# MiniMax-AI/VTP

Hardware: AMD Instinct MI355X
Metric: images/sec/node VTP-B f16d64 256x256 train step (higher is better)
Workload: dtype bf16

## Files before the change

### include/vtp_hip.h

```cpp
#ifndef VTP_HIP_H
#define VTP_HIP_H
#ifdef __cplusplus
extern "C" {
#endif

#define VTP_ABI_VERSION 1

int vtp_abi_version(void);
const char* vtp_last_error(void);

enum { VTP_EPI_BF16 = 0, VTP_EPI_F32 = 1, VTP_EPI_SWIGLU = 2, VTP_EPI_GELU = 3, VTP_EPI_F32_ATOMIC = 4, VTP_EPI_F32_SLAB = 5,
       VTP_EPI_QUICK_GELU = 8 };
int vtp_gemm_splits(int K, int splits);
int vtp_gemm_tn_splits(int M, int N, int K);
int vtp_gemm_tn(const void* A, int lda, const void* B, int ldb, void* C, int ldc, int ldc2, const float* resid, int M, int N,
                int K, int epilogue, int a_grp, int a_pre, int b_grp, int b_pre, int c_grp, int c_pre, int splits,
                float* a_colsum, void* stream);
int vtp_gemm_tn_grouped(const void* probs, int nprob, int ntiles, int K, int splits, void* part, void* ticket, void* stream);
int vtp_gemm_tn_grouped_limit(const void* probs, int nprob, int ntiles, int K, const int* k_rows, void* stream);
int vtp_gemm_tn_grouped_items(const void* probs, int nprob, int ntiles, int K, const void* items, int nitems, int slots, void* part,
                              void* ticket, void* stream);
int vtp_set_gemm_tuning(int force_cfg, int xcd_swizzle);
int vtp_set_gemm_dynamic(int on);
int vtp_gemm_debug(void* timing, int grid_limit, int delay_ticks);
// ... 139 lines not shown
int vtp_clip_grad_rows(const float* G, const float* B, const float* logit_scale, float* out, int M, int N, int D, int accumulate,
                       void* stream);
int vtp_clip_grad_cols(const float* G, const float* A, const float* logit_scale, float* out, int M, int N, int D, int accumulate,
                       void* stream);
int vtp_siglip_pairs(float* logits, const float* logit_bias, int B_local, int B_all, int label_offset, float weight,
                     float* loss_sum, float* d_logit_scale, float* d_logit_bias, void* stream);
int vtp_koleo(const float* xn, int* nn_scratch, float* d_xn, float* loss_sum, int B, int D, float weight, float eps, void* stream);
int vtp_sinkhorn_knopp(const void* logits, float inv_temp, void* probs, float* u, float* v, float* scratch, int T, int K, float count,
                       const float* count_dev, const int* n_rows_dev, int n_iters, int phase, void* stream);

int vtp_norm_fwd_e4m3(const float* x, const float* w, const float* b, void* y8, const float* q_scale, float* stats, int M, int D,
                      float eps, int kind, void* stream);
int vtp_quantize_e4m3(const void* src, int src_is_f32, void* dst, long n, const float* scale_dev, float scale, void* stream);
int vtp_amax(const void* src, int src_is_f32, long n, float* amax, void* stream);
int vtp_dequantize_e4m3(const void* src, float* dst, long n, float inv_scale, void* stream);
int vtp_gemm_nt_fp8(const void* A8, int lda, const void* B8, int ldb, void* C, int ldc, void* C2, int ldc2, const float* bias,
                    const float* resid, int M, int N, int K, int epilogue, float alpha, const int* rope_pos, const void* rope_sin,
                    const void* rope_cos, int rope_cols, void* stream);

int vtp_u8_to_images(const void* u8_nhwc, float* img_nchw, long B, int H, int W, const float* mean3, const float* std3, int flip,
                     void* stream);
int vtp_images_to_u8(const float* img_nchw, void* u8_nhwc, long B, int H, int W, const float* sub3, const float* div3, void* stream);
int vtp_latent_channel_stats(const float* latents, double* sums, long B, int C, int hw, void* stream);

int vtp_gather_token_rows(const void* src, const int* idx, void* dst, int T, int D, void* stream);
int vtp_scatter_token_rows(const void* d_dst, const int* idx, void* d_src, int T, int D, void* stream);
int vtp_weight_norm_prep(const float* v, const float* g, void* weff, void* weffT, float* inv_norm, int K, int C, void* stream);
int vtp_weight_norm_bwd(const float* dW, const float* v, const float* g, const float* inv_norm, float* dv, float* dg, int K, int C,
                        void* stream);
int vtp_softmax_center(const void* logits, const float* center, float inv_temp, void* probs, int T, int K, void* stream);
int vtp_softmax_center_dev(const void* logits, const float* center, const float* inv_temp, void* probs, int T, int K, void* stream);
int vtp_dino_ce(const void* student_logits, const void* teacher_probs, const int* t_idx0, const int* t_idx1,
                const float* row_weight, float inv_temp, float* loss_sum, void* d_student_logits, int T, int K, void* stream);
int vtp_center_ema(float* center, const float* col_sum, float inv_count, const float* count_ptr, float momentum, int K,
                   void* stream);

int vtp_conv3x3(const void* x, const void* w, const float* bias, void* y, const void* relu_mask, int NB, int H, int W, int Cin,
                int Cout, int taps, int mode, void* stream);
int vtp_lpips_unfold3(const void* tok, const float* img, void* out, int n, int H, int W, const float* shift, const float* scale,
                      void* stream);
int vtp_lpips_fold3_bwd(const void* dA, void* dt, int n, int H, int W, const float* scale, void* stream);
int vtp_maxpool2_fwd(const void* in, void* out, int NB, int H, int W, int C, void* stream);
int vtp_maxpool2_bwd(const void* Y, const void* dP, const void* tap, void* dY, int NB, int H, int W, int C, void* stream);
int vtp_lpips_tap(const void* f0, const void* f1, const float* w, float* val, void* df0, int n, int H, int W, int C,
                  float gscale, void* stream);

int vtp_probe_logits(const float* X, int ldx, const float* W, const float* bias, float* logits, int ldl, int B, int N, int K,
                     void* stream);
int vtp_probe_ce(const float* logits, int ldl, const long* labels, int B, int H, int C, float inv_rows, float* loss, int* correct,
                 float* dlogits, void* stream);
int vtp_probe_sgd(float* W, float* bias, float* mW, float* mb, const float* dlogits, int ldl, const float* X, int ldx, const float* lr,
                  int B, int H, int C, int K, float momentum, void* stream);

int vtp_zs_class_mean(const float* feat, int ldf, float* Wt, int ldw, int C, int T, int D, float eps, void* stream);
int vtp_zs_topk(const float* F, int ldf, const float* Wt, int ldw, const long* targets, float scale, int B, int C, int D,
                long* counts, int* per_class, int* rank, int* pred, float* logits, int ldl, void* stream);

int vtp_recon_scratch_doubles(long B, int H, int W);
int vtp_recon_metrics(const float* images, const float* recon, long B, int H, int W, const float* sub3, const float* div3,
                      void* ref_u8, void* rec_u8, float* ref_lp, float* rec_lp, double* scratch, long scratch_len, void* stream);
int vtp_recon_finalize(const double* scratch, long scratch_len, long B, int H, int W, float* psnr, float* ssim, double* sse,
                       const float* lpips, double* acc, void* stream);

int vtp_augment_scratch_floats(long N, int S);
int vtp_augment_crops(const void* src_u8, long B, int Hs, int Ws, const float* table, long N, int S, const float* mean3,
                      const float* std3, float* out, float* scratch, long scratch_len, void* stream);
// ... 68 lines not shown
```

### vtp_amd/_lib.py

```python
import ctypes
import os
from ctypes import c_char_p, c_float, c_int, c_long, c_void_p

_HERE = os.path.dirname(os.path.abspath(__file__))
LIB_PATH = os.environ.get("VTP_HIP_LIB") or os.path.join(_HERE, "lib", "libvtp_hip.so")

_P, _I, _L, _F = c_void_p, c_int, c_long, c_float

SIGNATURES = {
    "vtp_gemm_nt": [_P, _I, _P, _I, _P, _I, _P, _I, _P, _P, _P, _I, _I, _I, _I, _I, _I, _I, _I, _I, _F, _P],
    "vtp_norm_fwd": [_P, _P, _P, _P, _P, _I, _I, _F, _I, _P],
    "vtp_norm_bwd": [_P, _P, _P, _P, _P, _P, _P, _P, _P, _P, _I, _I, _I, _P],
    "vtp_norm_bwd_pvec": [_P, _P, _P, _P, _P, _P, _P, _P, _P, _P, _P, _I, _I, _I, _I, _I, _I, _P],
    "vtp_norm_bwd_rows": [_P, _P, _P, _P, _P, _P, _I, _P, _P, _P, _P, _P, _I, _I, _I, _P],
    "vtp_pool_patch_rows": [_P, _P, _I, _I, _I, _F, _P],
    "vtp_rope_qk": [_P, _P, _P, _I, _I, _I, _I, _I, _P],
    "vtp_attn_fwd": [_P, _P, _P, _P, _P, _I, _I, _I, _L, _L, _L, _L, _F, _I, _P],
    "vtp_attn_bwd": [_P, _P, _P, _P, _P, _P, _P, _P, _P, _P, _P, _P, _I, _I, _I, _I, _L, _L, _L, _L, _F, _I, _P],
    "vtp_im2col16": [_P, _P, _I, _I, _I, _P],
    "vtp_im2col16_rows": [_P, _P, _I, _I, _I, _I, _P],
    "vtp_col2im16": [_P, _P, _I, _I, _I, _P],
    "vtp_assemble_tokens": [_P, _P, _P, _P, _I, _I, _I, _P],
    "vtp_transpose_bf16": [_P, _I, _P, _I, _P, _I, _I, _I, _I, _I, _P],
    "vtp_strided_rowsum": [_P, _L, _P, _I, _I, _P],
# ... 23 lines not shown
    "vtp_colsum_bf16": [_P, _I, _P, _I, _I, _I, _I, _I, _P],
    "vtp_colsum_bf16_rows": [_P, _I, _P, _P, _I, _I, _P],
    "vtp_gather_image_rows": [_P, _P, _P, _P, _I, _L, _I, _F, _P],
    "vtp_scatter_image_rows": [_P, _P, _P, _I, _L, _I, _F, _I, _P],
    "vtp_gather_tail_rows": [_P, _P, _P, _P, _P, _I, _I, _I, _I, _P],
    "vtp_tail_row_map": [_P, _P, _I, _I, _I, _P],
    "vtp_expand_rows_bf16": [_P, _P, _P, _I, _I, _I, _P],
    "vtp_layerscale_wgrad": [_P, _P, _P, _P, _P, _P, _P, _P, _I, _I, _P],
    "vtp_scaled_transpose": [_P, _P, _P, _I, _I, _P],
    "vtp_qk_norm_fwd": [_P, _P, _P, _P, _P, _L, _I, _F, _P],
    "vtp_qk_norm_bwd": [_P, _P, _P, _P, _P, _P, _P, _L, _I, _P],
    "vtp_set_gemm_tuning": [_I, _I],
    "vtp_gemm_nt_config": [_I, _I, _I, _I],
    "vtp_gemm_debug": [_P, _I, _I],
    "vtp_attn_debug": [_P, _I, _I, _I],
    "vtp_cu_thief": [_I, _I, _P, _P],
    "vtp_set_gemm_dynamic": [_I],
    "vtp_norm_fwd_e4m3": [_P, _P, _P, _P, _P, _P, _I, _I, _F, _I, _P],
    "vtp_quantize_e4m3": [_P, _I, _P, _L, _P, _F, _P],
    "vtp_amax": [_P, _I, _L, _P, _P],
    "vtp_dequantize_e4m3": [_P, _P, _L, _F, _P],
    "vtp_gemm_nt_fp8": [_P, _I, _P, _I, _P, _I, _P, _I, _P, _P, _I, _I, _I, _I, _F, _P, _P, _P, _I, _P],
    "vtp_u8_to_images": [_P, _P, _L, _I, _I, _P, _P, _I, _P],
    "vtp_images_to_u8": [_P, _P, _L, _I, _I, _P, _P, _P],
    "vtp_latent_channel_stats": [_P, _P, _L, _I, _I, _P],
    "vtp_ema": [_P, _P, _L, _F, _P],
    "vtp_gather_token_rows": [_P, _P, _P, _I, _I, _P],
    "vtp_scatter_token_rows": [_P, _P, _P, _I, _I, _P],
    "vtp_weight_norm_prep": [_P, _P, _P, _P, _P, _I, _I, _P],
    "vtp_weight_norm_bwd": [_P, _P, _P, _P, _P, _P, _I, _I, _P],
    "vtp_softmax_center": [_P, _P, _F, _P, _I, _I, _P],
    "vtp_softmax_center_dev": [_P, _P, _P, _P, _I, _I, _P],
    "vtp_dino_ce": [_P, _P, _P, _P, _P, _F, _P, _P, _I, _I, _P],
    "vtp_center_ema": [_P, _P, _F, _P, _F, _I, _P],
    "vtp_conv3x3": [_P, _P, _P, _P, _P, _I, _I, _I, _I, _I, _I, _I, _P],
    "vtp_lpips_unfold3": [_P, _P, _P, _I, _I, _I, _P, _P, _P],
    "vtp_lpips_fold3_bwd": [_P, _P, _I, _I, _I, _P, _P],
    "vtp_maxpool2_fwd": [_P, _P, _I, _I, _I, _I, _P],
    "vtp_maxpool2_bwd": [_P, _P, _P, _P, _I, _I, _I, _I, _P],
    "vtp_lpips_tap": [_P, _P, _P, _P, _P, _I, _I, _I, _I, _F, _P],
    "vtp_ema_dev": [_P, _P, _L, _P, _P],
    "vtp_adamw_ema_dev": [_P, _P, _P, _P, _P, _P, _L, _P, _P],
    "vtp_adamw_dev_grouped": [_P, _P, _P, _P, _P, _P, _P, _I, _L, _P, _P],
    "vtp_adamw_ema_dev_grouped": [_P, _P, _P, _P, _P, _P, _P, _I, _L, _P, _P],
    "vtp_sumsq_partials_count": [_L],
    "vtp_sumsq_partials": [_P, _L, _P, _P],
    "vtp_sum_partials": [_P, _I, _P, _P],
    "vtp_grad_clip_finalize": [_P, _I, _P, _P, _P, _P],
    "vtp_grad_clip_finalize_guarded": [_P, _I, _P, _P, _P, _P, _P, _P],
    "vtp_adamw_dev_guarded": [_P, _P, _P, _P, _P, _P, _P, _I, _L, _P, _P, _P],
    "vtp_adamw_ema_dev_guarded": [_P, _P, _P, _P, _P, _P, _P, _I, _L, _P, _P, _P],
    "vtp_ema_dev_guarded": [_P, _P, _L, _P, _P, _P],
    "vtp_embed_tokens": [_P, _P, _P, _P, _P, _I, _I, _I, _P],
    "vtp_embed_tokens_bwd": [_P, _P, _P, _P, _I, _I, _I, _P],
    "vtp_gather_rows": [_P, _P, _P, _I, _I, _I, _P],
    "vtp_scatter_rows": [_P, _P, _P, _P, _I, _I, _I, _P],
    "vtp_text_row_plan": [_P, _P, _P, _P, _I, _I, _P],
    "vtp_embed_tokens_packed": [_P, _P, _P, _P, _P, _I, _I, _I, _P],
    "vtp_embed_tokens_bwd_packed": [_P, _P, _P, _P, _P, _I, _I, _I, _P],
    "vtp_gather_rows_packed": [_P, _P, _P, _I, _I, _P],
    "vtp_scatter_rows_packed": [_P, _P, _P, _P, _I, _I, _I, _P],
    "vtp_gelu_bwd_limit": [_P, _P, _P, _I, _I, _I, _P, _P],
    "vtp_norm_fwd_limit": [_P, _P, _P, _P, _P, _I, _I, _F, _I, _P, _P],
    "vtp_norm_bwd_limit": [_P, _P, _P, _P, _P, _P, _P, _P, _P, _P, _I, _I, _I, _P, _P],
    "vtp_gemm_nt_limit": [_P, _I, _P, _I, _P, _I, _P, _I, _P, _P, _P, _I, _I, _I, _I, _F, _P, _P],
    "vtp_attn_fwd_varlen": [_P, _P, _P, _P, _P, _P, _I, _I, _I, _L, _L, _F, _P],
# ... 92 lines not shown
```

### vtp_amd/csrc/ssl.hip

```cpp
#include "common.h"
#include "vtp_hip.h"

namespace vtp {

__global__ __launch_bounds__(256) void gather_token_rows_kernel(const bf16* __restrict__ src, const int* __restrict__ idx,
                                                                bf16* __restrict__ dst, int T, int D) {
  const int d8 = D / 8;
  const long total = (long)T * d8;
  for (long i = blockIdx.x * 256L + threadIdx.x; i < total; i += (long)gridDim.x * 256L) {
    const int t = (int)(i / d8), c = (int)(i % d8);
    const int r = idx[t];
    bf16x8 v;
    if (r >= 0) {
      v = *(const bf16x8*)(src + (long)r * D + 8 * c);
    } else {
#pragma unroll
      for (int e = 0; e < 8; ++e) v[e] = (bf16)0.f;
    }
    *(bf16x8*)(dst + (long)t * D + 8 * c) = v;
  }
}

__global__ __launch_bounds__(256) void scatter_token_rows_kernel(const bf16* __restrict__ d_dst, const int* __restrict__ idx,
                                                                 bf16* __restrict__ d_src, int T, int D) {
// ... 26 lines not shown
    if (weffT) weffT[(long)c * K + k] = w;
  }
  if (lane == 0) inv_norm[k] = inv;
}

__global__ __launch_bounds__(256) void weight_norm_prep_tiled_kernel(const float* __restrict__ v, const float* __restrict__ g,
                                                                     bf16* __restrict__ weff, bf16* __restrict__ weffT,
                                                                     float* __restrict__ inv_norm, int K, int C) {
  __shared__ bf16 tile[64][256 + 2];
  const int lane = threadIdx.x & 63, wave = threadIdx.x >> 6;
  const int k0 = blockIdx.x * 64;
  for (int r = wave; r < 64; r += 4) {
    const int k = k0 + r;
    if (k >= K) break;
    float s = 0.f;
    for (int c = lane; c < C; c += 64) {
      const float x = v[(long)k * C + c];
      s += x * x;
    }
    s = wave_sum(s);
    const float inv = rsqrtf(s);
    const float sc = g[k] * inv;
    for (int c = lane; c < C; c += 64) {
      const bf16 w = f2bf(v[(long)k * C + c] * sc);
      weff[(long)k * C + c] = w;
      tile[r][c] = w;
    }
    if (lane == 0) inv_norm[k] = inv;
  }
  __syncthreads();
  const int k = k0 + lane;
  if (k < K)
    for (int c = wave; c < C; c += 4) weffT[(long)c * K + k] = tile[lane][c];
}

__global__ __launch_bounds__(256) void weight_norm_bwd_kernel(const float* __restrict__ dW, const float* __restrict__ v,
                                                              const float* __restrict__ g, const float* __restrict__ inv_norm,
                                                              float* __restrict__ dv, float* __restrict__ dg, int K, int C) {
  const int lane = threadIdx.x & 63;
  const int k = blockIdx.x * 4 + (threadIdx.x >> 6);
  if (k >= K) return;
  const float inv = inv_norm[k];
  float dot = 0.f;
  for (int c = lane; c < C; c += 64) dot += dW[(long)k * C + c] * v[(long)k * C + c] * inv;
  dot = wave_sum(dot);
  const float sc = g[k] * inv;
  for (int c = lane; c < C; c += 64) {
    const float vh = v[(long)k * C + c] * inv;
    dv[(long)k * C + c] += sc * (dW[(long)k * C + c] - dot * vh);
  }
  if (lane == 0) dg[k] += dot;
}

__device__ __forceinline__ void row_lse(const bf16* __restrict__ row, const float* __restrict__ center, float sc, int K,
                                        float* red, float& mx_out, float& se_out) {
  float mx = -INFINITY, se = 0.f;
  for (int k = threadIdx.x * 8; k < K; k += 256 * 8) {
    bf16x8 v = *(const bf16x8*)(row + k);
#pragma unroll
    for (int e = 0; e < 8; ++e) {
      const float x = (bf2f(v[e]) - (center ? center[k + e] : 0.f)) * sc;
      if (x > mx) {
        se = se * __expf(mx - x) + 1.f;
        mx = x;
      } else {
        se += __expf(x - mx);
      }
    }
  }
#pragma unroll
  for (int o = 32; o > 0; o >>= 1) {
    const float m2 = __shfl_xor(mx, o, 64), s2 = __shfl_xor(se, o, 64);
    const float m = fmaxf(mx, m2);
    se = (mx == -INFINITY ? 0.f : se * __expf(mx - m)) + (m2 == -INFINITY ? 0.f : s2 * __expf(m2 - m));
    mx = m;
  }
  const int w = threadIdx.x >> 6;
  __syncthreads();
  if ((threadIdx.x & 63) == 0) {
    red[2 * w] = mx;
    red[2 * w + 1] = se;
  }
  __syncthreads();
  float m = fmaxf(fmaxf(red[0], red[2]), fmaxf(red[4], red[6]));
  float s = 0.f;
#pragma unroll
// ... 97 lines not shown
  if (wr == 0.f || i0 < 0) {
    for (int k = threadIdx.x * 8; k < K; k += 256 * 8) {
      bf16x8 z;
#pragma unroll
      for (int e = 0; e < 8; ++e) z[e] = (bf16)0.f;
      *(bf16x8*)(drow + k) = z;
    }
    return;
  }
  float mx, se;
  row_lse(row, nullptr, inv_temp, K, red, mx, se);
  const float lse = mx + __logf(se);
  const float nt = i1 >= 0 ? 2.f : 1.f;
  const bf16* p0 = P + (long)i0 * K;
  const bf16* p1 = i1 >= 0 ? P + (long)i1 * K : nullptr;
  float loss = 0.f;
  for (int k = threadIdx.x * 8; k < K; k += 256 * 8) {
    bf16x8 s = *(const bf16x8*)(row + k), a = *(const bf16x8*)(p0 + k), b, o;
    if (p1) b = *(const bf16x8*)(p1 + k);
#pragma unroll
    for (int e = 0; e < 8; ++e) {
      const float lsm = bf2f(s[e]) * inv_temp - lse;
      const float q = bf2f(a[e]) + (p1 ? bf2f(b[e]) : 0.f);
      loss -= q * lsm;
      o[e] = f2bf(wr * inv_temp * (nt * __expf(lsm) - q));
    }
    *(bf16x8*)(drow + k) = o;
  }
  __shared__ float red2[4];
  loss = block_sum<4>(loss, red2);
  if (threadIdx.x == 0) unsafeAtomicAdd(loss_sum, wr * loss);
}

__global__ __launch_bounds__(256) void center_ema_kernel(float* __restrict__ center, const float* __restrict__ col_sum,
                                                         float inv_count, const float* __restrict__ count_ptr, float momentum,
                                                         int K) {
  const int k = blockIdx.x * 256 + threadIdx.x;
  if (count_ptr) inv_count = 1.f / fmaxf(count_ptr[0], 1.f);
  if (k < K) center[k] = momentum * center[k] + (1.f - momentum) * col_sum[k] * inv_count;
}

}
using namespace vtp;

static inline int ssl_grid(long items) {
  long b = (items + 255) / 256;
  return (int)(b > 4096 ? 4096 : (b < 1 ? 1 : b));
}

extern "C" int vtp_gather_token_rows(const void* src, const int* idx, void* dst, int T, int D, void* stream) {
  VTP_REQUIRE(src && idx && dst && T > 0 && D > 0 && D % 8 == 0, "vtp_gather_token_rows: bad argument (D %% 8 == 0)");
  hipLaunchKernelGGL(gather_token_rows_kernel, dim3(ssl_grid((long)T * D / 8)), dim3(256), 0, (hipStream_t)stream,
                     (const bf16*)src, idx, (bf16*)dst, T, D);
  return check_launch("gather_token_rows");
}

extern "C" int vtp_scatter_token_rows(const void* d_dst, const int* idx, void* d_src, int T, int D, void* stream) {
  VTP_REQUIRE(d_dst && idx && d_src && T > 0 && D > 0 && D % 8 == 0, "vtp_scatter_token_rows: bad argument (D %% 8 == 0)");
  hipLaunchKernelGGL(scatter_token_rows_kernel, dim3(ssl_grid((long)T * D / 8)), dim3(256), 0, (hipStream_t)stream,
                     (const bf16*)d_dst, idx, (bf16*)d_src, T, D);
  return check_launch("scatter_token_rows");
}

extern "C" int vtp_weight_norm_prep(const float* v, const float* g, void* weff, void* weffT, float* inv_norm, int K, int C,
                                    void* stream) {
  VTP_REQUIRE(v && g && weff && inv_norm && K > 0 && C > 0, "vtp_weight_norm_prep: bad argument");
  if (weffT && C <= 256)
    hipLaunchKernelGGL(weight_norm_prep_tiled_kernel, dim3(cdiv(K, 64)), dim3(256), 0, (hipStream_t)stream, v, g, (bf16*)weff,
                       (bf16*)weffT, inv_norm, K, C);
  else
    hipLaunchKernelGGL(weight_norm_prep_kernel, dim3(cdiv(K, 4)), dim3(256), 0, (hipStream_t)stream, v, g, (bf16*)weff,
                       (bf16*)weffT, inv_norm, K, C);
  return check_launch("weight_norm_prep");
}

extern "C" int vtp_weight_norm_bwd(const float* dW, const float* v, const float* g, const float* inv_norm, float* dv, float* dg,
                                   int K, int C, void* stream) {
  VTP_REQUIRE(dW && v && g && inv_norm && dv && dg && K > 0 && C > 0, "vtp_weight_norm_bwd: bad argument");
  hipLaunchKernelGGL(weight_norm_bwd_kernel, dim3(cdiv(K, 4)), dim3(256), 0, (hipStream_t)stream, dW, v, g, inv_norm, dv, dg, K, C);
  return check_launch("weight_norm_bwd");
}

static int launch_softmax_center(const void* logits, const float* center, float inv_temp, const float* inv_temp_dev, void* probs, int T,
                                 int K, void* stream) {
  if (K <= 65536 && K >= 8192)
    hipLaunchKernelGGL(softmax_center_reg_kernel, dim3(T), dim3(1024), 0, (hipStream_t)stream, (const bf16*)logits, center,
                       inv_temp, (bf16*)probs, K, inv_temp_dev);
  else
    hipLaunchKernelGGL(softmax_center_kernel, dim3(T), dim3(256), 0, (hipStream_t)stream, (const bf16*)logits, center, inv_temp,
                       (bf16*)probs, K, inv_temp_dev);
  return check_launch("softmax_center");
}

extern "C" int vtp_softmax_center(const void* logits, const float* center, float inv_temp, void* probs, int T, int K,
                                  void* stream) {
  VTP_REQUIRE(logits && probs && T > 0 && K > 0 && K % 8 == 0, "vtp_softmax_center: bad argument (K %% 8 == 0)");
  return launch_softmax_center(logits, center, inv_temp, nullptr, probs, T, K, stream);
}

extern "C" int vtp_softmax_center_dev(const void* logits, const float* center, const float* inv_temp, void* probs, int T, int K,
                                      void* stream) {
  VTP_REQUIRE(logits && probs && inv_temp && T > 0 && K > 0 && K % 8 == 0, "vtp_softmax_center_dev: bad argument (K %% 8 == 0)");
  return launch_softmax_center(logits, center, 0.f, inv_temp, probs, T, K, stream);
}

extern "C" int vtp_dino_ce(const void* student_logits, const void* teacher_probs, const int* t_idx0, const int* t_idx1,
                           const float* row_weight, float inv_temp, float* loss_sum, void* d_student_logits, int T, int K,
                           void* stream) {
  VTP_REQUIRE(student_logits && teacher_probs && t_idx0 && t_idx1 && row_weight && loss_sum && d_student_logits,
              "vtp_dino_ce: null pointer");
  VTP_REQUIRE(T > 0 && K > 0 && K % 8 == 0, "vtp_dino_ce: bad shape (K %% 8 == 0)");
  hipLaunchKernelGGL(dino_ce_kernel, dim3(T), dim3(256), 0, (hipStream_t)stream, (const bf16*)student_logits,
                     (const bf16*)teacher_probs, t_idx0, t_idx1, row_weight, inv_temp, loss_sum, (bf16*)d_student_logits, K);
  return check_launch("dino_ce");
}

extern "C" int vtp_center_ema(float* center, const float* col_sum, float inv_count, const float* count_ptr, float momentum,
                              int K, void* stream) {
  VTP_REQUIRE(center && col_sum && K > 0, "vtp_center_ema: bad argument");
  hipLaunchKernelGGL(center_ema_kernel, dim3(cdiv(K, 256)), dim3(256), 0, (hipStream_t)stream, center, col_sum, inv_count,
                     count_ptr, momentum, K);
  return check_launch("center_ema");
}
```

### vtp_amd/ops.py

```python
from __future__ import annotations

import torch

from . import _lib

EPI_BF16, EPI_F32, EPI_SWIGLU, EPI_GELU, EPI_F32_ATOMIC, EPI_F32_SLAB = 0, 1, 2, 3, 4, 5
EPI_QUICK_GELU = 8
NORM_RMS, NORM_LN = 0, 1


def _s():
    return torch.cuda.current_stream().cuda_stream


def _p(t):
    return 0 if t is None else t.data_ptr()


def _lib_():
    return _lib.load()


def pad8(n: int) -> int:
    return (n + 7) // 8 * 8
# ... 497 lines not shown
def sinkhorn_knopp(logits, inv_temp, probs, u, v, scratch, T, K, count, n_iters=3, phase=-1, count_dev=None, n_rows_dev=None):
    _lib.check(_lib_().vtp_sinkhorn_knopp(_p(logits), inv_temp, _p(probs), _p(u), _p(v), _p(scratch), T, K, float(count), _p(count_dev),
                                          _p(n_rows_dev), n_iters, phase, _s()), "vtp_sinkhorn_knopp")


def gather_token_rows(src, idx, dst, T, D):
    _lib.check(_lib_().vtp_gather_token_rows(_p(src), _p(idx), _p(dst), T, D, _s()), "vtp_gather_token_rows")


def scatter_token_rows(d_dst, idx, d_src, T, D):
    _lib.check(_lib_().vtp_scatter_token_rows(_p(d_dst), _p(idx), _p(d_src), T, D, _s()), "vtp_scatter_token_rows")


def weight_norm_prep(v, g, weff, weffT, inv_norm, K, C):
    _lib.check(_lib_().vtp_weight_norm_prep(_p(v), _p(g), _p(weff), _p(weffT), _p(inv_norm), K, C, _s()), "vtp_weight_norm_prep")


def weight_norm_bwd(dW, v, g, inv_norm, dv, dg, K, C):
    _lib.check(_lib_().vtp_weight_norm_bwd(_p(dW), _p(v), _p(g), _p(inv_norm), _p(dv), _p(dg), K, C, _s()), "vtp_weight_norm_bwd")


def softmax_center(logits, center, inv_temp, probs, T, K):
    if isinstance(inv_temp, torch.Tensor):
        _lib.check(_lib_().vtp_softmax_center_dev(_p(logits), _p(center), _p(inv_temp), _p(probs), T, K, _s()), "vtp_softmax_center_dev")
    else:
        _lib.check(_lib_().vtp_softmax_center(_p(logits), _p(center), inv_temp, _p(probs), T, K, _s()), "vtp_softmax_center")


def dino_ce(s_logits, t_probs, t0, t1, w, inv_temp, loss_sum, d_logits, T, K):
    _lib.check(_lib_().vtp_dino_ce(_p(s_logits), _p(t_probs), _p(t0), _p(t1), _p(w), inv_temp, _p(loss_sum), _p(d_logits), T, K,
                                   _s()), "vtp_dino_ce")


def center_ema(center, col_sum, inv_count, momentum, K, count=None):
    _lib.check(_lib_().vtp_center_ema(_p(center), _p(col_sum), inv_count, _p(count), momentum, K, _s()), "vtp_center_ema")


def ema_dev(t, s, n, momentum_dev):
    _lib.check(_lib_().vtp_ema_dev(_p(t), _p(s), n, _p(momentum_dev), _s()), "vtp_ema_dev")


def adamw_ema_dev(p, g, m, v, teacher, n, hyper, nodecay4=None):
    _lib.check(_lib_().vtp_adamw_ema_dev(_p(p), _p(g), _p(m), _p(v), _p(teacher), _p(nodecay4), n, _p(hyper), _s()), "vtp_adamw_ema_dev")



def adamw_dev_grouped(p, g, m, v, p_bf16, n, hyper, group4, group_tab, ngroups):
    _lib.check(_lib_().vtp_adamw_dev_grouped(_p(p), _p(g), _p(m), _p(v), _p(p_bf16), _p(group4), _p(group_tab), ngroups, n, _p(hyper),
                                             _s()), "vtp_adamw_dev_grouped")


def adamw_ema_dev_grouped(p, g, m, v, teacher, n, hyper, group4, group_tab, ngroups):
    _lib.check(_lib_().vtp_adamw_ema_dev_grouped(_p(p), _p(g), _p(m), _p(v), _p(teacher), _p(group4), _p(group_tab), ngroups, n,
                                                 _p(hyper), _s()), "vtp_adamw_ema_dev_grouped")


def sumsq_partials_count(n: int) -> int:
    return int(_lib_().vtp_sumsq_partials_count(n))


def sumsq_partials(g, n, partials):
    _lib.check(_lib_().vtp_sumsq_partials(_p(g), n, _p(partials), _s()), "vtp_sumsq_partials")


def sum_partials(partials, count, out):
    _lib.check(_lib_().vtp_sum_partials(_p(partials), count, _p(out), _s()), "vtp_sum_partials")
# ... 615 lines not shown
```

### vtp_amd/train.py

```python
from __future__ import annotations

import math
import os
from typing import List, Optional, Sequence, Tuple

import torch

from . import ops
from .engine import BF, F32, OVERLAP


class GradBucketer:

    def __init__(self, flat_g: torch.Tensor, group=None, shard: bool = False, grad_dtype: torch.dtype = torch.float32,
                 force: bool = False):
        import torch.distributed as dist
        self.dist = dist
        self.flat_g = flat_g
        self.group = group
        self.world = dist.get_world_size(group) if dist.is_available() and dist.is_initialized() else 1
        self.rank = dist.get_rank(group) if self.world > 1 else 0
        self.active = self.world > 1 or (bool(force) and dist.is_available() and dist.is_initialized())
        self.works = []
        self.reduced_elems = 0
# ... 355 lines not shown
        if no_decay is not None:
            flags = torch.zeros(st.numel // 4, dtype=torch.uint8)
            for name, (o, k) in st.offsets.items():
                if no_decay(name, tuple(st.params[name].shape)):
                    flags[o // 4:(o + (k + 3) // 4 * 4) // 4] = 1
            self.nodecay4 = flags.to(st.device)
        self.param_groups = self.group_tab = self._group4 = self._group_ring = None
        if param_groups is not None:
            shapes = {name: tuple(st.params[name].shape) for name in st.offsets}
            self.param_groups, rows = resolve_param_groups(param_groups, shapes, no_decay)
            idx = torch.zeros(st.numel // 4, dtype=torch.uint8)
            for name, (o, k) in st.offsets.items():
                idx[o // 4:(o + (k + 3) // 4 * 4) // 4] = rows[name]
            self._group4 = idx.to(st.device)
            self.group_tab = torch.tensor(group_table(self.param_groups), dtype=F32, device=st.device).view(-1, 2)
        self.step_no = 0
        self.loss_sum = torch.zeros(1, dtype=F32, device=st.device)
        self.clip_loss_sum = torch.zeros(1, dtype=F32, device=st.device)
        if shard_optimizer is None:
            shard_optimizer = os.environ.get("VTP_SHARD_OPT", "0") == "1"
        if grad_dtype not in ("fp32", "bf16"):
            raise ValueError(f"grad_dtype must be 'fp32' or 'bf16', got {grad_dtype!r}")
        if grad_dtype == "bf16" and not shard_optimizer:
            raise ValueError("grad_dtype='bf16' needs shard_optimizer=True (the all-reduce path reduces the flat fp32 buffer in place)")
        self.bucketer = GradBucketer(st.flat_g, group, shard=shard_optimizer, grad_dtype=BF if grad_dtype == "bf16" else F32,
                                     force=force_collectives)
        self.shard_optimizer = self.bucketer.shard
        self._shard_layout = None
        self.overlap_opt = (not self.shard_optimizer) and os.environ.get("VTP_OPT_OVERLAP", "1") not in ("0", "false", "off")
        self._opt_stream = self._zero_stream = None
        self._opt_plans = {}
        self._opt_busy = self._zero_busy = False
        self.head_overlap = os.environ.get("VTP_HEAD_OVERLAP", "1") not in ("0", "false", "off")
        self._head_stream, self._head_keys = None, []
        self._works_prev = []
        self.collectives = self.bucketer.active
        if self.collectives:
            from . import _lib
            _lib.load().vtp_set_gemm_dynamic(1)
        self.time_comm = False
        self._comm_events = []
        self.world, self.rank, self.group = self.bucketer.world, self.bucketer.rank, group
        for eng in self._aug_engines():
            eng.rope_aug.reseed(drop_seed, self.rank)
        self._graph_aug = {}
        self.bucket_blocks = bucket_blocks
        self._bucket_plan = self._plan_buckets()
        self.hyper = torch.zeros(16, dtype=F32, device=st.device)
        self.momentum_dev = self.hyper[9:10]
        self._clip = max_grad_norm is not None
        self._max_grad_norm = _max_norm_value(max_grad_norm) if self._clip else None
        self.grad_norm = self.grad_clip_coef = self._clip_partials = self._clip_sum = None
        self._clip_ranges, self._clip_cursor, self._clip_keys = {}, 0, []
        if self._clip:
            self.grad_norm = torch.zeros(1, dtype=F32, device=st.device)
            self.grad_clip_coef = torch.zeros(1, dtype=F32, device=st.device)
            cap = ops.sumsq_partials_count(st.numel) + len(st.offsets)
            self._clip_partials = torch.zeros(cap, dtype=torch.float64, device=st.device)
            self._clip_sum = torch.zeros(1, dtype=torch.float64, device=st.device)
        self._skip_state = self.step_skipped = self.skipped_steps = None
        if self._skip:
            self._skip_state = torch.zeros(4, dtype=torch.int32, device=st.device)
            self.skipped_steps = self._skip_state[1:2]
            self.step_skipped = self._skip_state[2:3]
        self._hyper_ring = None
        self.use_graphs = use_graphs
# ... 81 lines not shown
        return result

    def _ssl_gen(self, P, lead_images=None):
        from .vtp import ssl_forward
        out = ssl_forward(self.model, P["global"], P["local"], P["masks"], P["plan"], P["dev"], train=True, lead_images=lead_images,
                          tail_rows="student_tail_src" in P["dev"])
        self._zero_join()
        if not (self.head_overlap and not self.collectives and OVERLAP.enabled):
            yield from self._ssl_tail(out, P)
            return out
        main = torch.cuda.current_stream()
        self.trunk.d_xnf_buffer(out["ctx"]).zero_()
        if self._head_stream is None:
            self._head_stream = torch.cuda.Stream()
        self._head_stream.wait_stream(main)
        with torch.cuda.stream(self._head_stream), OVERLAP.lane(2):
            was, OVERLAP.enabled = OVERLAP.enabled, False
            try:
                for ev in self._ssl_tail(out, P, zero_dxnf=False):
                    if callable(ev):
                        raise RuntimeError("head stream: the SSL tail asked for a collective")
                    self._head_keys += ev
            finally:
                OVERLAP.enabled = was
        return out

    def _ssl_tail(self, out, P, zero_dxnf: bool = True):
        model, st, head = self.model, self.store, self.ssl_head
        dist = self.bucketer.dist
        K, D = head.K, self.trunk.D
        Tt, Ts, Tm, B2, nl = out["Tt"], out["Ts"], out["Tm"], out["B2"], out["nl"]
        ws = out["ws"]
        t_logits, s_logits = out["teacher_logits"], out["student_logits"]
        probs = ws.get("probs", (Tt, K), BF)
        if self.centering == "sinkhorn_knopp":
            yield from self._sinkhorn_targets(ws, t_logits, probs, P, B2, Tm, K)
        else:
            inv_tt = self.hyper[8:9]
            ops.softmax_center(t_logits, self.center_dino, inv_tt, probs, B2, K)
            ops.softmax_center(t_logits[B2:], self.center_ibot, inv_tt, probs[B2:], Tm, K)
            stats = self.center_stats
            stats.zero_()
            ops.colsum_bf16(t_logits, K, stats, B2, K)
            ops.colsum_bf16_rows(t_logits[B2:], K, stats[K:], P["dev"]["n_masked_i"], Tm, K)
            stats[2 * K:2 * K + 1].copy_(P["dev"]["n_masked_f"])

            def apply_centers():
                ops.center_ema(self.center_dino, stats, 1.0 / (B2 * self.world), self.center_momentum, K)
                ops.center_ema(self.center_ibot, stats[K:], 0.0, self.center_momentum, K, count=stats[2 * K:])
            if self.collectives:
                yield lambda: self.bucketer.works.append((dist.all_reduce(stats, group=self.group, async_op=True), None))
                self._deferred.append(apply_centers)
            else:
                apply_centers()
        d_logits = ws.get("d_logits", (Ts, K), BF)
        ops.dino_ce(s_logits, probs, P["dev"]["t0"], P["dev"]["t1"], P["dev"]["w"], 1.0 / self.student_temp, self.ssl_loss_sum,
                    d_logits, Ts, K)
        dX = head.backward(d_logits, out["head_ctx"])
        if self.koleo_weight > 0:
            self._koleo(ws, out["Hs"], dX, nl, B2, head.Din)
        yield ["dino_head"]
        from .vtp import ssl_head_input_bwd
        dX = ssl_head_input_bwd(model, out, dX)
        ctx = out["ctx"]
        d_xnf = self.trunk.d_xnf_buffer(ctx)
        if zero_dxnf:
            d_xnf.zero_()
        if out["tail"] is not None:
            ops.gather_token_rows(dX, P["dev"]["student_tail_keep"], d_xnf[out["tail"]:], Ts, D)
            return
        seg_g, seg_l = ctx.segs[-2], ctx.segs[-1]
        ops.scatter_token_rows(dX, P["dev"]["student_local_src"], d_xnf[seg_l.row0:], nl, D)
        ops.scatter_token_rows(dX[nl:], P["dev"]["student_global_src"], d_xnf[seg_g.row0:], Ts - nl, D)

    def _sinkhorn_targets(self, ws, t_logits, probs, P, B2, Tm, K):
        dist = self.bucketer.dist
        it = self.sk_iterations
        inv_t = 1.0 / self.teacher_temp
        for tag, lg, pr, T, cnt_dev, rows_dev, count in (("cls", t_logits, probs, B2, None, None, float(B2 * self.world)),
                                                         ("patch", t_logits[B2:], probs[B2:], Tm, P["dev"]["n_masked_f"],
                                                          P["dev"]["n_masked_i"], 0.0)):
            u, v = ws.get(f"sk.u.{tag}", (T,), F32), ws.get(f"sk.v.{tag}", (K,), F32)
            scr = ws.get(f"sk.s.{tag}", (8 + K + T,), F32)
            if not self.collectives:
                ops.sinkhorn_knopp(lg, inv_t, pr, u, v, scr, T, K, count, it, -1, cnt_dev, rows_dev)
                continue
            if cnt_dev is not None:
                gcnt = ws.get("sk.cnt", (1,), F32)
                gcnt.copy_(cnt_dev)
                yield lambda gcnt=gcnt: dist.all_reduce(gcnt, group=self.group)
# ... 767 lines not shown
```

Measured before the change: 760.7.

## Fuse iBOT teacher softmax into CE kernel and add row-wise weight-norm kernels

Adds a fused iBOT cross-entropy kernel that computes the centered teacher softmax inline per masked-token row, instead of first writing a probs buffer for the masked tokens and reading it back in the CE pass. DINO CLS rows still go through the existing softmax_center and dino_ce. It also adds new weight-norm prep and backward kernels that process several rows per wave, stage the transpose through LDS, and use vector stores. The weight-norm kernels are on by default for C<=256 and can be turned off by environment variable. This cuts HBM traffic and kernel launches in the SSL head, at the cost of high register pressure from a 1024-thread kernel that holds 64 logits per thread.

New measurement: 767.2 (median of 6 runs). No clear change (+0.9%).

```diff
diff --git a/include/vtp_hip.h b/include/vtp_hip.h
--- a/include/vtp_hip.h
+++ b/include/vtp_hip.h
@@ -195,6 +195,9 @@
 int vtp_softmax_center_dev(const void* logits, const float* center, const float* inv_temp, void* probs, int T, int K, void* stream);
 int vtp_dino_ce(const void* student_logits, const void* teacher_probs, const int* t_idx0, const int* t_idx1,
                 const float* row_weight, float inv_temp, float* loss_sum, void* d_student_logits, int T, int K, void* stream);
+int vtp_ibot_ce_fused(const void* student_logits, const void* teacher_logits, const float* center, const float* teacher_inv_temp,
+                      const int* t_idx0, const float* row_weight, float inv_temp, float* loss_sum, void* d_student_logits, int T,
+                      int K, void* stream);
 int vtp_center_ema(float* center, const float* col_sum, float inv_count, const float* count_ptr, float momentum, int K,
                    void* stream);
 
diff --git a/vtp_amd/_lib.py b/vtp_amd/_lib.py
--- a/vtp_amd/_lib.py
+++ b/vtp_amd/_lib.py
@@ -79,6 +79,7 @@
     "vtp_softmax_center": [_P, _P, _F, _P, _I, _I, _P],
     "vtp_softmax_center_dev": [_P, _P, _P, _P, _I, _I, _P],
     "vtp_dino_ce": [_P, _P, _P, _P, _P, _F, _P, _P, _I, _I, _P],
+    "vtp_ibot_ce_fused": [_P, _P, _P, _P, _P, _P, _F, _P, _P, _I, _I, _P],
     "vtp_center_ema": [_P, _P, _F, _P, _F, _I, _P],
     "vtp_conv3x3": [_P, _P, _P, _P, _P, _I, _I, _I, _I, _I, _I, _I, _P],
     "vtp_lpips_unfold3": [_P, _P, _P, _I, _I, _I, _P, _P, _P],
diff --git a/vtp_amd/csrc/ssl.hip b/vtp_amd/csrc/ssl.hip
--- a/vtp_amd/csrc/ssl.hip
+++ b/vtp_amd/csrc/ssl.hip
@@ -82,6 +82,73 @@
   const int k = k0 + lane;
   if (k < K)
     for (int c = wave; c < C; c += 4) weffT[(long)c * K + k] = tile[lane][c];
+}
+
+constexpr int WN_ROWS = 128, WN_LD = WN_ROWS + 4;
+__global__ __launch_bounds__(256) void weight_norm_prep_rows_kernel(const float* __restrict__ v, const float* __restrict__ g,
+                                                                    bf16* __restrict__ weff, bf16* __restrict__ weffT,
+                                                                    float* __restrict__ inv_norm, int K, int C) {
+  __shared__ __attribute__((aligned(16))) bf16 tile[256 * WN_LD];
+  const int lane = threadIdx.x & 63, wave = threadIdx.x >> 6;
+  const int k0 = blockIdx.x * WN_ROWS;
+  const int kw = k0 + wave * (WN_ROWS / 4);
+  float x[2][4][4];
+  auto load4 = [&](int b, int kb) {
+#pragma unroll
+    for (int i = 0; i < 4; ++i)
+#pragma unroll
+      for (int j = 0; j < 4; ++j) {
+        const int c = lane + 64 * j;
+        x[b][i][j] = (kb + i < K && c < C) ? v[(long)(kb + i) * C + c] : 0.f;
+      }
+  };
+  load4(0, kw);
+#pragma unroll
+  for (int it = 0; it < WN_ROWS / 16; ++it) {
+    const int kb = kw + 4 * it, b = it & 1;
+    if (it + 1 < WN_ROWS / 16) load4(b ^ 1, kb + 4);
+    float s[4];
+#pragma unroll
+    for (int i = 0; i < 4; ++i) {
+      s[i] = 0.f;
+#pragma unroll
+      for (int j = 0; j < 4; ++j) s[i] += x[b][i][j] * x[b][i][j];
+    }
+#pragma unroll
+    for (int o = 32; o > 0; o >>= 1)
+#pragma unroll
+      for (int i = 0; i < 4; ++i) s[i] += __shfl_xor(s[i], o, 64);
+#pragma unroll
+    for (int i = 0; i < 4; ++i) {
+      const int k = kb + i;
+      if (k >= K) break;
+      const float inv = rsqrtf(s[i]);
+      const float sc = g[k] * inv;
+#pragma unroll
+      for (int j = 0; j < 4; ++j) {
+        const int c = lane + 64 * j;
+        if (c < C) {
+          const bf16 w = f2bf(x[b][i][j] * sc);
+          weff[(long)k * C + c] = w;
+          tile[c * WN_LD + (k - k0)] = w;
+        }
+      }
+      if (lane == 0) inv_norm[k] = inv;
+    }
+  }
+  __syncthreads();
+  const int kq = 4 * (threadIdx.x & 31), k = k0 + kq;
+  const bool vec = (K & 3) == 0;
+  if (k < K)
+    for (int c = threadIdx.x >> 5; c < C; c += 8) {
+      const bf16* t = tile + c * WN_LD + kq;
+      bf16* o = weffT + (long)c * K + k;
+      if (vec) {
+        *(bf16x4*)o = *(const bf16x4*)t;
+      } else {
+        for (int e = 0; e < 4 && k + e < K; ++e) o[e] = t[e];
+      }
+    }
 }
 
 __global__ __launch_bounds__(256) void weight_norm_bwd_kernel(const float* __restrict__ dW, const float* __restrict__ v,
@@ -102,6 +169,55 @@
   if (lane == 0) dg[k] += dot;
 }
 
+__global__ __launch_bounds__(256) void weight_norm_bwd_rows_kernel(const float* __restrict__ dW, const float* __restrict__ v,
+                                                                   const float* __restrict__ g, const float* __restrict__ inv_norm,
+                                                                   float* __restrict__ dv, float* __restrict__ dg, int K, int C) {
+  const int lane = threadIdx.x & 63;
+  const int kb = (blockIdx.x * 4 + (threadIdx.x >> 6)) * 4;
+  float a[4][4], x[4][4], d[4][4], inv[4], dot[4];
+#pragma unroll
+  for (int i = 0; i < 4; ++i) {
+    const bool row = kb + i < K;
+    inv[i] = row ? inv_norm[kb + i] : 0.f;
+#pragma unroll
+    for (int j = 0; j < 4; ++j) {
+      const int c = lane + 64 * j;
+      const bool in = row && c < C;
+      const long at = (long)(kb + i) * C + c;
+      a[i][j] = in ? dW[at] : 0.f;
+      x[i][j] = in ? v[at] : 0.f;
+      d[i][j] = in ? dv[at] : 0.f;
+    }
+  }
+#pragma unroll
+  for (int i = 0; i < 4; ++i) {
+    dot[i] = 0.f;
+#pragma unroll
+    for (int j = 0; j < 4; ++j)
+      if (lane + 64 * j < C) dot[i] += a[i][j] * x[i][j] * inv[i];
+  }
+#pragma unroll
+  for (int o = 32; o > 0; o >>= 1)
+#pragma unroll
+    for (int i = 0; i < 4; ++i) dot[i] += __shfl_xor(dot[i], o, 64);
+#pragma unroll
+  for (int i = 0; i < 4; ++i) {
+    const int k = kb + i;
+    if (k >= K) break;
+    const float sc = g[k] * inv[i];
+#pragma unroll
+    for (int j = 0; j < 4; ++j) {
+      const int c = lane + 64 * j;
+      if (c < C) {
+        const float vh = x[i][j] * inv[i];
+        d[i][j] += sc * (a[i][j] - dot[i] * vh);
+        dv[(long)k * C + c] = d[i][j];
+      }
+    }
+    if (lane == 0) dg[k] += dot[i];
+  }
+}
+
 __device__ __forceinline__ void row_lse(const bf16* __restrict__ row, const float* __restrict__ center, float sc, int K,
                                         float* red, float& mx_out, float& se_out) {
   float mx = -INFINITY, se = 0.f;
@@ -265,6 +381,163 @@
   if (threadIdx.x == 0) unsafeAtomicAdd(loss_sum, wr * loss);
 }
 
+template <bool CENTER, bool FULL>
+__global__ __launch_bounds__(1024) void ibot_ce_fused_kernel(const bf16* __restrict__ S, const bf16* __restrict__ T,
+                                                             const float* __restrict__ center,
+                                                             const float* __restrict__ inv_temp_t_dev, const int* __restrict__ t0,
+                                                             const float* __restrict__ w, float inv_temp,
+                                                             float* __restrict__ loss_sum, bf16* __restrict__ dS, int K) {
+  __shared__ float red[64];
+  const int r = blockIdx.x;
+  bf16* drow = dS + (long)r * K;
+  const float wr = w[r];
+  const int i0 = t0[r];
+  if (wr == 0.f || i0 < 0) {
+    bf16x8 zero;
+#pragma unroll
+    for (int e = 0; e < 8; ++e) zero[e] = (bf16)0.f;
+    for (int k = threadIdx.x * 8; k < K; k += 1024 * 8) *(bf16x8*)(drow + k) = zero;
+    return;
+  }
+  const float inv_tt = *inv_temp_t_dev;
+  const bf16* srow = S + (long)r * K;
+  const bf16* trow = T + (long)i0 * K;
+  const int w16 = threadIdx.x >> 6, lane = threadIdx.x & 63;
+  const int t8 = threadIdx.x * 8;
+  float z[8][8];
+  float mx = -INFINITY;
+  bool in[8];
+  bf16x8 v[8];
+#pragma unroll
+  for (int c = 0; c < 8; ++c) {
+    in[c] = FULL || c * 8192 + t8 < K;
+    v[c] = *(const bf16x8*)(trow + (in[c] ? c * 8192 + t8 : 0));
+  }
+#pragma unroll
+  for (int h = 0; h < 2; ++h) {
+    f32x4 c0[4], c1[4];
+#pragma unroll
+    for (int i = 0; i < 4; ++i) {
+      const int c = 4 * h + i;
+      c0[i] = f32x4{0.f, 0.f, 0.f, 0.f};
+      c1[i] = c0[i];
+      if (CENTER) {
+        const int k = in[c] ? c * 8192 + t8 : 0;
+        c0[i] = *(const f32x4*)(center + k);
+        c1[i] = *(const f32x4*)(center + k + 4);
+      }
+    }
+    __builtin_amdgcn_sched_barrier(0);
+#pragma unroll
+    for (int i = 0; i < 4; ++i) {
+      const int c = 4 * h + i;
+#pragma unroll
+      for (int e = 0; e < 8; ++e) {
+        z[c][e] = in[c] ? (bf2f(v[c][e]) - (e < 4 ? c0[i][e] : c1[i][e - 4])) * inv_tt : -INFINITY;
+        mx = fmaxf(mx, z[c][e]);
+      }
+    }
+    __builtin_amdgcn_sched_barrier(0);
+  }
+  bf16x8 s[8];
+  auto load_student = [&]() {
+#pragma unroll
+    for (int c = 0; c < 8; ++c) {
+      s[c] = *(const bf16x8*)(srow + (in[c] ? c * 8192 + t8 : 0));
+      if (!in[c]) {
+#pragma unroll
+        for (int e = 0; e < 8; ++e) s[c][e] = (bf16)(-INFINITY);
+      }
+    }
+    __builtin_amdgcn_sched_barrier(0);
+  };
+  if (FULL) load_student();
+  mx = wave_max(mx);
+  if (lane == 0) red[w16] = mx;
+  __syncthreads();
+  mx = red[0];
+#pragma unroll
+  for (int i = 1; i < 16; ++i) mx = fmaxf(mx, red[i]);
+  float se = 0.f;
+#pragma unroll
+  for (int c = 0; c < 8; ++c)
+#pragma unroll
+    for (int e = 0; e < 8; ++e) {
+      z[c][e] = __expf(z[c][e] - mx);
+      se += z[c][e];
+    }
+  se = wave_sum(se);
+  if (lane == 0) red[16 + w16] = se;
+  __syncthreads();
+  se = 0.f;
+#pragma unroll
+  for (int i = 0; i < 16; ++i) se += red[16 + i];
+  const float inv = 1.f / se;
+  bf16x8 p[8];
+#pragma unroll
+  for (int c = 0; c < 8; ++c)
+#pragma unroll
+    for (int e = 0; e < 8; ++e) p[c][e] = f2bf(z[c][e] * inv);
+#pragma unroll
+  for (int c = 0; c < 8; ++c) asm volatile("" : "+v"(p[c]));
+  __builtin_amdgcn_sched_barrier(0);
+  if (!FULL) load_student();
+#pragma unroll
+  for (int c = 0; c < 8; ++c) asm volatile("" : "+v"(s[c]));
+  mx = -INFINITY;
+#pragma unroll
+  for (int c = 0; c < 8; ++c)
+#pragma unroll
+    for (int e = 0; e < 8; ++e) mx = fmaxf(mx, bf2f(s[c][e]) * inv_temp);
+  mx = wave_max(mx);
+  if (lane == 0) red[32 + w16] = mx;
+  __syncthreads();
+  mx = red[32];
+#pragma unroll
+  for (int i = 1; i < 16; ++i) mx = fmaxf(mx, red[32 + i]);
+  se = 0.f;
+#pragma unroll
+  for (int c = 0; c < 8; ++c) asm volatile("" : "+v"(s[c]));
+#pragma unroll
+  for (int c = 0; c < 8; ++c)
+#pragma unroll
+    for (int e = 0; e < 8; ++e) se += __expf(bf2f(s[c][e]) * inv_temp - mx);
+  se = wave_sum(se);
+  if (lane == 0) red[48 + w16] = se;
+  __syncthreads();
+  se = 0.f;
+#pragma unroll
+  for (int i = 0; i < 16; ++i) se += red[48 + i];
+  const float lse = mx + __logf(se);
+  const float nt = 1.f;
+  float loss = 0.f;
+#pragma unroll
+  for (int c = 0; c < 8; ++c) asm volatile("" : "+v"(s[c]));
+#pragma unroll
+  for (int c = 0; c < 8; ++c) {
+    if (in[c]) {
+      bf16x8 o;
+#pragma unroll
+      for (int e = 0; e < 8; ++e) {
+        const float lsm = bf2f(s[c][e]) * inv_temp - lse;
+        const float q = bf2f(p[c][e]);
+        loss -= q * lsm;
+        o[e] = f2bf(wr * inv_temp * (nt * __expf(lsm) - q));
+      }
+      *(bf16x8*)(drow + c * 8192 + t8) = o;
+    }
+  }
+  loss = wave_sum(loss);
+  if (lane == 0) red[w16] = loss;
+  __syncthreads();
+  if (threadIdx.x == 0) {
+    float t = 0.f;
+#pragma unroll
+    for (int i = 0; i < 16; ++i) t += red[i];
+    unsafeAtomicAdd(loss_sum, wr * t);
+  }
+}
+
 __global__ __launch_bounds__(256) void center_ema_kernel(float* __restrict__ center, const float* __restrict__ col_sum,
                                                          float inv_count, const float* __restrict__ count_ptr, float momentum,
                                                          int K) {
@@ -295,10 +568,18 @@
   return check_launch("scatter_token_rows");
 }
 
+static inline bool wnorm_rows() {
+  const char* e = getenv("VTP_WNORM_PREP");
+  return !(e && e[0] == '0');
+}
+
 extern "C" int vtp_weight_norm_prep(const float* v, const float* g, void* weff, void* weffT, float* inv_norm, int K, int C,
                                     void* stream) {
   VTP_REQUIRE(v && g && weff && inv_norm && K > 0 && C > 0, "vtp_weight_norm_prep: bad argument");
-  if (weffT && C <= 256)
+  if (weffT && C <= 256 && wnorm_rows())
+    hipLaunchKernelGGL(weight_norm_prep_rows_kernel, dim3(cdiv(K, WN_ROWS)), dim3(256), 0, (hipStream_t)stream, v, g, (bf16*)weff,
+                       (bf16*)weffT, inv_norm, K, C);
+  else if (weffT && C <= 256)
     hipLaunchKernelGGL(weight_norm_prep_tiled_kernel, dim3(cdiv(K, 64)), dim3(256), 0, (hipStream_t)stream, v, g, (bf16*)weff,
                        (bf16*)weffT, inv_norm, K, C);
   else
@@ -310,7 +591,11 @@
 extern "C" int vtp_weight_norm_bwd(const float* dW, const float* v, const float* g, const float* inv_norm, float* dv, float* dg,
                                    int K, int C, void* stream) {
   VTP_REQUIRE(dW && v && g && inv_norm && dv && dg && K > 0 && C > 0, "vtp_weight_norm_bwd: bad argument");
-  hipLaunchKernelGGL(weight_norm_bwd_kernel, dim3(cdiv(K, 4)), dim3(256), 0, (hipStream_t)stream, dW, v, g, inv_norm, dv, dg, K, C);
+  if (C <= 256 && wnorm_rows())
+    hipLaunchKernelGGL(weight_norm_bwd_rows_kernel, dim3(cdiv(K, 16)), dim3(256), 0, (hipStream_t)stream, dW, v, g, inv_norm, dv, dg,
+                       K, C);
+  else
+    hipLaunchKernelGGL(weight_norm_bwd_kernel, dim3(cdiv(K, 4)), dim3(256), 0, (hipStream_t)stream, dW, v, g, inv_norm, dv, dg, K, C);
   return check_launch("weight_norm_bwd");
 }
 
@@ -348,6 +633,19 @@
   return check_launch("dino_ce");
 }
 
+extern "C" int vtp_ibot_ce_fused(const void* student_logits, const void* teacher_logits, const float* center,
+                                 const float* teacher_inv_temp, const int* t_idx0, const float* row_weight, float inv_temp,
+                                 float* loss_sum, void* d_student_logits, int T, int K, void* stream) {
+  VTP_REQUIRE(student_logits && teacher_logits && teacher_inv_temp && t_idx0 && row_weight && loss_sum && d_student_logits,
+              "vtp_ibot_ce_fused: null pointer");
+  VTP_REQUIRE(T > 0 && K > 0 && K % 8 == 0 && K <= 65536, "vtp_ibot_ce_fused: bad shape (K %% 8 == 0, K <= 65536)");
+  auto kern = K == 65536 ? (center ? ibot_ce_fused_kernel<true, true> : ibot_ce_fused_kernel<false, true>)
+                         : (center ? ibot_ce_fused_kernel<true, false> : ibot_ce_fused_kernel<false, false>);
+  hipLaunchKernelGGL(kern, dim3(T), dim3(1024), 0, (hipStream_t)stream, (const bf16*)student_logits, (const bf16*)teacher_logits,
+                     center, teacher_inv_temp, t_idx0, row_weight, inv_temp, loss_sum, (bf16*)d_student_logits, K);
+  return check_launch("ibot_ce_fused");
+}
+
 extern "C" int vtp_center_ema(float* center, const float* col_sum, float inv_count, const float* count_ptr, float momentum,
                               int K, void* stream) {
   VTP_REQUIRE(center && col_sum && K > 0, "vtp_center_ema: bad argument");
diff --git a/vtp_amd/ops.py b/vtp_amd/ops.py
--- a/vtp_amd/ops.py
+++ b/vtp_amd/ops.py
@@ -553,6 +553,15 @@
                                    _s()), "vtp_dino_ce")
 
 
+def ibot_ce_fused(s_logits, t_logits, center, t_inv_temp, t0, w, inv_temp, loss_sum, d_logits, T, K):
+    _lib.check(_lib_().vtp_ibot_ce_fused(_p(s_logits), _p(t_logits), _p(center), _p(t_inv_temp), _p(t0), _p(w), inv_temp,
+                                         _p(loss_sum), _p(d_logits), T, K, _s()), "vtp_ibot_ce_fused")
+
+
+def ibot_ce_fused_fits(K):
+    return K % 8 == 0 and K <= 65536
+
+
 def center_ema(center, col_sum, inv_count, momentum, K, count=None):
     _lib.check(_lib_().vtp_center_ema(_p(center), _p(col_sum), inv_count, _p(count), momentum, K, _s()), "vtp_center_ema")
 
diff --git a/vtp_amd/train.py b/vtp_amd/train.py
--- a/vtp_amd/train.py
+++ b/vtp_amd/train.py
@@ -411,6 +411,7 @@
         self._opt_plans = {}
         self._opt_busy = self._zero_busy = False
         self.head_overlap = os.environ.get("VTP_HEAD_OVERLAP", "1") not in ("0", "false", "off")
+        self.ibot_fused = os.environ.get("VTP_IBOT_FUSED", "1") not in ("0", "false", "off")
         self._head_stream, self._head_keys = None, []
         self._works_prev = []
         self.collectives = self.bucketer.active
@@ -558,13 +559,23 @@
         Tt, Ts, Tm, B2, nl = out["Tt"], out["Ts"], out["Tm"], out["B2"], out["nl"]
         ws = out["ws"]
         t_logits, s_logits = out["teacher_logits"], out["student_logits"]
-        probs = ws.get("probs", (Tt, K), BF)
+        fused = self.ibot_fused and self.centering != "sinkhorn_knopp" and ops.ibot_ce_fused_fits(K)
+        probs = ws.get("probs", (B2 if fused else Tt, K), BF)
+        d_logits = ws.get("d_logits", (Ts, K), BF)
         if self.centering == "sinkhorn_knopp":
             yield from self._sinkhorn_targets(ws, t_logits, probs, P, B2, Tm, K)
         else:
             inv_tt = self.hyper[8:9]
             ops.softmax_center(t_logits, self.center_dino, inv_tt, probs, B2, K)
-            ops.softmax_center(t_logits[B2:], self.center_ibot, inv_tt, probs[B2:], Tm, K)
+            if fused:
+                n_cls = nl + B2
+                dev = P["dev"]
+                ops.dino_ce(s_logits, probs, dev["t0"], dev["t1"], dev["w"], 1.0 / self.student_temp, self.ssl_loss_sum, d_logits,
+                            n_cls, K)
+                ops.ibot_ce_fused(s_logits[n_cls:], t_logits, self.center_ibot, inv_tt, dev["t0"][n_cls:], dev["w"][n_cls:],
+                                  1.0 / self.student_temp, self.ssl_loss_sum, d_logits[n_cls:], Tm, K)
+            else:
+                ops.softmax_center(t_logits[B2:], self.center_ibot, inv_tt, probs[B2:], Tm, K)
             stats = self.center_stats
             stats.zero_()
             ops.colsum_bf16(t_logits, K, stats, B2, K)
@@ -579,9 +590,9 @@
                 self._deferred.append(apply_centers)
             else:
                 apply_centers()
-        d_logits = ws.get("d_logits", (Ts, K), BF)
-        ops.dino_ce(s_logits, probs, P["dev"]["t0"], P["dev"]["t1"], P["dev"]["w"], 1.0 / self.student_temp, self.ssl_loss_sum,
-                    d_logits, Ts, K)
+        if not fused:
+            ops.dino_ce(s_logits, probs, P["dev"]["t0"], P["dev"]["t1"], P["dev"]["w"], 1.0 / self.student_temp, self.ssl_loss_sum,
+                        d_logits, Ts, K)
         dX = head.backward(d_logits, out["head_ctx"])
         if self.koleo_weight > 0:
             self._koleo(ws, out["Hs"], dX, nl, B2, head.Din)
```
